# google/libultrahdr

Measured on AMD Instinct MI355X. Metric: Mpixels/s encode+decode (API-1 P010+YUV420, 4K), device-resident round trip, higher is better.
Workload: dtype f32; 1 GPU; API-1 3840x2160 round trip per step: encode (P010 HLG + YCbCr420 -> two-pass 3-ch gain map at scale 1, FDCT q95, Huffman: two JPEG scans) + decode (Huffman, IDCT, applyGainMap -> RGBA_F16 linear); frames resident in HBM

## Files before the change

libultrahdr_amd/csrc/api_entropy.cpp:

```cpp
#include "api_internal.h"

#include <condition_variable>
#include <functional>
#include <mutex>

uhdr_error_info_t uhdr_api::check_scan(const uhdr_hip_jpeg_scan_t* sc, bool need_coef, int* mcus_per_row, int* mcu_rows, int* blocks_per_mcu) {
  if (!sc) return err_status(UHDR_CODEC_INVALID_PARAM, "received nullptr for the scan description");
  if (sc->num_components != 1 && sc->num_components != 3)
    return err_status(UHDR_CODEC_INVALID_PARAM, "a scan has 1 or 3 components, received %d", sc->num_components);
  if (sc->w == 0 || sc->h == 0 || sc->w > 65535 || sc->h > 65535)
    return err_status(UHDR_CODEC_INVALID_PARAM, "image dimensions %ux%u are outside JPEG's 1..65535", sc->w, sc->h);
  int hmax = 1, vmax = 1, bpm = 0;
  for (int i = 0; i < sc->num_components; i++) {
    const int hs = sc->num_components == 1 ? 1 : sc->h_samp[i], vs = sc->num_components == 1 ? 1 : sc->v_samp[i];
    if (hs < 1 || hs > 2 || vs < 1 || vs > 2) return err_status(UHDR_CODEC_INVALID_PARAM, "component %d: sampling factors %dx%d not in {1, 2}", i, hs, vs);
    if (hs > hmax) hmax = hs;
    if (vs > vmax) vmax = vs;
    bpm += hs * vs;
    if (need_coef && (!sc->coef[i] || ((uintptr_t)sc->coef[i] & 15)))
      return err_status(UHDR_CODEC_INVALID_PARAM, "coefficient buffer %d is null or not 16-byte aligned", i);
    if (sc->blocks_w[i] < 1 || sc->blocks_h[i] < 1) return err_status(UHDR_CODEC_INVALID_PARAM, "component %d: empty block grid", i);
  }
  if (bpm > 10) return err_status(UHDR_CODEC_INVALID_PARAM, "an MCU holds at most 10 blocks (T.81 B.2.3), received %d", bpm);
  if (sc->num_components == 1) {
// ... 315 lines not shown
      if (n != 0 && !(n & 0x8000u) && (int)((n >> 8) & 31u) <= r) second = v_ac[next9];
    }
    out[2 * idx] = first;
    out[2 * idx + 1] = second;
  }
}

uhdr_error_info_t uhdr_hip_huffman_decode_dev(uhdr_hip_ctx_t* c, const uhdr_hip_jpeg_scan_t* sc, const uhdr_hip_huff_tables_t* tables,
                                              const uint8_t* data, size_t data_bytes) {
  if (!c) return err_status(UHDR_CODEC_INVALID_PARAM, "received nullptr for uhdr_hip context");
  if (!data || data_bytes == 0 || data_bytes > 0xFFFFFFF0ull) return err_status(UHDR_CODEC_INVALID_PARAM, "received no (or more than 4 GiB of) entropy-coded data");
  int mpr = 0, mrows = 0, bpm = 0;
  UHDR_TRY(check_scan(sc, true, &mpr, &mrows, &bpm));
  if (sc->restart_interval < 0 || sc->restart_interval > 65535) return err_status(UHDR_CODEC_INVALID_PARAM, "restart_interval %d out of range", sc->restart_interval);
  HIP_TRY(hipSetDevice(c->device));
  if (!c->d_huff) {
    std::vector<uint32_t> blob(host::jpeg_huff_code_tables());
    blob.resize((size_t)host::kHuffTabWords + 16);
    memcpy(blob.data() + host::kHuffTabWords, host::jpeg_zigzag_to_natural(), 64);
    HIP_TRY(hipMalloc((void**)&c->d_huff, blob.size() * sizeof(uint32_t)));
    HIP_TRY(hipMemcpyAsync(c->d_huff, blob.data(), blob.size() * sizeof(uint32_t), hipMemcpyHostToDevice, c->stream));
    HIP_TRY(hipStreamSynchronize(c->stream));
  }
  const DbgClock dbg;
  constexpr size_t kTabDec = 0, kTabFast = (sizeof(HuffDecTable) * 4 + 255) & ~(size_t)255,
                   kTabVal = (kTabFast + sizeof(HuffFastTable) * 8 + 255) & ~(size_t)255, kTabPair = kTabVal + (size_t)4 * kHuffValWords * 4,
                   kTabPairVal = kTabPair + (size_t)kHuffPairBlobWords * 4, kTabBytes = kTabPairVal + (size_t)kHuffPairValBlobWords * 4;
  {
    uint8_t key[4 * (17 + 256)];
    for (int t = 0; t < 4; t++) {
// ... 155 lines not shown
    const size_t o_sl = use_hyp ? take((size_t)nsub * (size_t)bpm * 8) : 0;
    const int max_pieces = [&] {
      const char* e = getenv("UHDR_HIP_HUFF_PIECES");
      const int v = e ? atoi(e) : 4;
      return (use_hyp && form2 && !rst_sync && v >= 1 && v <= 4) ? v : 1;
    }();
    const size_t o_ms = max_pieces > 1 ? take((size_t)nsub * kHuffHypSlots * (size_t)(max_pieces - 1) * 8) : 0;
    const size_t o_mc = max_pieces > 1 ? take((size_t)nsub * kHuffHypSlots * (size_t)(max_pieces - 1) * 2) : 0;
    const size_t o_pe = max_pieces > 1 ? take((size_t)nsub * (size_t)max_pieces * 8 + 64) : 0;
    const size_t o_pc = max_pieces > 1 ? take(((size_t)nsub * (size_t)max_pieces + 4) * 4) : 0;
    const size_t o_st2 = max_pieces > 1 ? take(((size_t)nsub * (size_t)max_pieces / 2048 + 4) * 4) : 0;
    const bool form3 = jblock_ok && attempts[0].levels > 0;
    const bool scratch2 = form2 && !form3;
    const size_t scan_bytes = scratch2 ? (size_t)total_blocks * 64 * sizeof(int16_t) : 0;
    const size_t o_cs = scratch2 ? take(scan_bytes + 256) : 0;
    UHDR_TRY(ensure(c->scratch[6], off));
    uint8_t* sb = (uint8_t*)c->scratch[6].p;
    HuffSyncArgs y;
    memset(&y, 0, sizeof y);
    y.clean = sb + o_clean;
    y.nbytes = (uint32_t)data_bytes;
    y.flags = (uint32_t*)(sb + o_flags);
    y.nstuffed = y.flags + 8;
    y.sub_bits = sub_bits;
    y.state[0] = (uint64_t*)(sb + o_s0); y.state[1] = (uint64_t*)(sb + o_s1);
    y.changed[0] = sb + o_c0; y.changed[1] = sb + o_c1;
    y.nblk = (uint32_t*)(sb + o_nblk);
    y.scan_tmp = (uint32_t*)(sb + o_st);
    y.dcd = (int*)(sb + o_dcd);
    y.total_blocks = total_blocks;
// ... 13 lines not shown
      y.first_blk[i] = j;
      for (int k = 0; k < a.hs[i] * a.vs[i] && j < 16; k++) y.comp_of[j++] = (uint8_t)i;
    }
    y.ftabs = (const HuffFastTable*)(tabs_dev + kTabFast);
    y.ttabs = y.ftabs + 4;
    y.vtabs = (const uint32_t*)(tabs_dev + kTabVal);
    y.ptabs = (const uint32_t*)(tabs_dev + kTabPair);
    y.pvtabs = (const uint32_t*)(tabs_dev + kTabPairVal);
    y.zigzag = a.zigzag;
    (void)o_ft; (void)o_vt;
    if (use_hyp) {
      y.strag_list = (uint32_t*)(sb + o_sl);
      y.strag_cap = nsub * (uint32_t)bpm;
    }
    if (scratch2) y.coef_scan = (int16_t*)(sb + o_cs);
    y.total_mcus = (uint32_t)a.total_mcus;
    const int main_levels_env = [&] { const char* e = getenv("UHDR_HIP_HUFF_MAIN_LEVELS"); return e ? atoi(e) : (sparse ? 1 : 2); }();
    if (j == bpm && bpm <= 16) {
      const bool fills_in_unstuff = attempts[0].levels > 0 && zero_bytes_sync % 16 == 0 && ff_bytes % 16 == 0 && zero_bytes_sync / 16 < 0xFFFFFFFFull &&
                                    ff_bytes / 16 < 0xFFFFFFFFull && !getenv("UHDR_HIP_HUFF_FILL_LAUNCHES");
      HuffInitFill init_fill;
      memset(&init_fill, 0, sizeof init_fill);
      if (fills_in_unstuff) {
        init_fill.zero_ptr = (uint4*)y.flags;
        init_fill.zero_vec = (uint32_t)(zero_bytes_sync / 16);
        init_fill.ff_ptr = (uint4*)y.state[0];
        init_fill.ff_vec = (uint32_t)(ff_bytes / 16);
      } else {
        HIP_TRY(hipMemsetAsync(y.flags, 0, zero_bytes_sync, c->stream));
      }
// ... 99 lines not shown
            fprintf(stderr, "uhdr_hip: rounds decode of %zu bytes, %u subsequences of %u bits (write form %d): %s\n", data_bytes, nsub_t, t.sub_bits,
                    y.coef_scan && !rst_sync ? 2 : 1, fl[4 + max_rounds % 3] == 0 ? "settled" : "NOT settled");
        }
      }
      const bool settled = hyp_done || fl[4 + max_rounds % 3] == 0;
      if (rst_sync && getenv("UHDR_HIP_HUFF_DEBUG"))
        fprintf(stderr, "uhdr_hip: restart file through the parallel decoder: %s, status bits %#x, %u markers dropped (%d expected), sequence sums %s\n",
                settled ? "settled" : "NOT settled", fl[1], fl[9], a.nseg - 1, fl[0] == fl[16] && fl[7] == fl[17] ? "equal" : "DIFFERENT");
      if (settled && rst_sync && ((fl[1] & 14u) != 0 || fl[9] != (uint32_t)(a.nseg - 1) || fl[0] != fl[16] || fl[7] != fl[17])) {
        for (int i = 0; i < a.ncomp; i++) HIP_TRY(hipMemsetAsync(a.coef[i], 0, zero_bytes[i], c->stream));
        coef_zeroed = true;
      } else if (settled) {
        if (fl[1] & 8u) return err_status(UHDR_CODEC_INVALID_PARAM, "corrupt entropy-coded data (the scan ends before its last block)");
        if (fl[1] & 2u) return err_status(UHDR_CODEC_INVALID_PARAM, "corrupt entropy-coded data (undefined Huffman code or a run past the end of a block)");
        sync_done = true;
      } else {
        if (a.nseg == 1 && !c->huff_serial_ok && data_bytes > (256u << 10)) {
          c->stats.entropy_decode_declined++;
          return err_status(UHDR_CODEC_UNSUPPORTED_FEATURE, "the parallel entropy decode did not settle in %d rounds; %zu bytes on one lane would take longer than the CPU", max_rounds, data_bytes);
        }
        for (int i = 0; i < a.ncomp; i++) HIP_TRY(hipMemsetAsync(a.coef[i], 0, zero_bytes[i], c->stream));
        coef_zeroed = true;
      }
    }
  }
  if (sync_done) {
    c->stats.entropy_decode_parallel++;
    return ok_status();
  }
  if (a.nseg == 1 && !c->huff_serial_ok && data_bytes > (256u << 10)) {
// ... 194 lines not shown
```

libultrahdr_amd/csrc/api_internal.h:

```cpp
#ifndef UHDR_HIP_API_INTERNAL_H
#define UHDR_HIP_API_INTERNAL_H

#pragma GCC visibility push(default)
#include "uhdr_hip.h"
#pragma GCC visibility pop

#include <cfloat>
#include <chrono>
#include <cmath>
#include <cstdarg>
#include <cstdio>
#include <cstring>
#include <atomic>
#include <functional>
#include <map>
#include <memory>
#include <string>
#include <thread>
#include <vector>
#include "exact_math.h"
#include "host_tables.h"
#include "uhdr_types.h"
#include "rccl_bind.h"

// ... 63 lines not shown
  float* d_pq_buckets = nullptr;
  float* d_hlg_buckets_pre = nullptr;
  float* d_pq_buckets_pre = nullptr;
  float* d_hlg_inv_ootf = nullptr;
  double* d_math = nullptr;
  float* h_tab[kTableSlots] = {};
  float* d_tab[kTableSlots] = {};
  size_t tab_cap[kTableSlots] = {};
  hipEvent_t tab_ev[kTableSlots] = {};
  std::string tab_key[kTableSlots];
  size_t tab_gamma_off[kTableSlots] = {};
  int tab_next = 0;
  DeviceBuf scratch[8];
  uhdr_hip_stats_t stats = {};
  bool huff_serial_ok = true;
  DeviceBuf huff_slots;
  bool huff_two_pass = false;
  bool huff_route_log = false;
  size_t huff_slots_refused = 0;
  DeviceBuf enc[3];
  uhdr_hip_ctx* aux = nullptr;
  struct AuxWorker* aux_worker = nullptr;
  DeviceBuf jpg[6];
  struct Resident {
    DeviceBuf buf;
    bool valid = false;
    uhdr_img_fmt_t fmt = UHDR_IMG_FMT_UNSPECIFIED;
    unsigned int w = 0, h = 0;
    const void* host[3] = {};
    unsigned int host_stride[3] = {};
// ... 146 lines not shown
```

libultrahdr_amd/csrc/api_jpeg.cpp:

```cpp
#include "api_internal.h"

void uhdr_hip_jpeg_quant_table(int quality, int is_chroma, uint16_t qt[64]) { host::jpeg_quant_table(quality, is_chroma, qt); }

int uhdr_hip_oetf_code_thresholds(uhdr_color_transfer_t ct, float thresholds[1024]) {
  if ((ct != UHDR_CT_HLG && ct != UHDR_CT_PQ) || !thresholds) return -1;
  const std::vector<float>& t = host::oetf_code_thresholds(ct);
  for (int i = 0; i < 1024; i++) thresholds[i] = t[(size_t)i];
  return 0;
}

uhdr_error_info_t uhdr_hip_selftest(uhdr_hip_ctx_t* c, int which, unsigned int arg0, unsigned int arg1, unsigned int seed, const float mm[6],
                                    unsigned long long out[8]) {
  if (!c) return err_status(UHDR_CODEC_INVALID_PARAM, "received nullptr for uhdr_hip context");
  if (!out || which < 0 || which > 7 || (which == 5 && !mm) || (which == 6 && (!mm || arg0 > 1)) ||
      ((which == 4 || which == 7) && (!mm || arg0 > 2 || arg1 < 1 || arg1 > 3 || arg0 >= arg1)) || (which == 2 && (arg0 < 1 || arg1 > 254 || arg0 > arg1)))
    return err_status(UHDR_CODEC_INVALID_PARAM, "bad self-test arguments");
  HIP_TRY(hipSetDevice(c->device));
  UHDR_TRY(upload_math(c));
  UHDR_TRY(ensure(c->affine, kAffineDevBytes));
  UHDR_TRY(ensure(c->exchange, 256));
  unsigned long long* d_out = (unsigned long long*)c->exchange.p;
  HIP_TRY(hipMemsetAsync(d_out, 0, 64, c->stream));
  if (which == 4) {
    MinmaxTableParams t;
// ... 979 lines not shown

uhdr_error_info_t uhdr_hip_jpeg_ycc_to_rgb(uhdr_hip_ctx_t* c, const uhdr_raw_image_t* ycc, int variant, uhdr_raw_image_t* rgb) {
  if (!c) return err_status(UHDR_CODEC_INVALID_PARAM, "received nullptr for uhdr_hip context");
  UHDR_TRY(check_jpeg_color(rgb, ycc, false));
  HIP_TRY(hipSetDevice(c->device));
  uhdr_raw_image_t tmp = *rgb;
  tmp.w = ycc->w; tmp.h = ycc->h;
  uhdr_raw_image_t ds, dd;
  UHDR_TRY(stage_in(c, 0, ycc, &ds, true));
  UHDR_TRY(stage_in(c, 1, &tmp, &dd, false));
  UHDR_TRY(uhdr_hip_jpeg_ycc_to_rgb_dev(c, &ds, variant, &dd));
  rgb->cg = dd.cg; rgb->ct = dd.ct; rgb->range = dd.range; rgb->w = dd.w; rgb->h = dd.h;
  return stage_out(c, &dd, rgb);
}

uhdr_error_info_t uhdr_hip_idct_dequant_rgb_dev(uhdr_hip_ctx_t* c, const int16_t* coef_y, const int16_t* coef_cb, const int16_t* coef_cr,
                                                int bw, int bh, const uint16_t qt_luma[64], const uint16_t qt_chroma[64], int variant,
                                                uhdr_raw_image_t* rgb) {
  if (!c) return err_status(UHDR_CODEC_INVALID_PARAM, "received nullptr for uhdr_hip context");
  if (!coef_y || !coef_cb || !coef_cr || !qt_luma || !qt_chroma || !rgb || !rgb->planes[0] || bw <= 0 || bh <= 0)
    return err_status(UHDR_CODEC_INVALID_PARAM, "received bad argument for idct_dequant_rgb");
  if (rgb->fmt != UHDR_IMG_FMT_24bppRGB888 && rgb->fmt != UHDR_IMG_FMT_32bppRGBA8888)
    return err_status(UHDR_CODEC_UNSUPPORTED_FEATURE, "idct_dequant_rgb expects UHDR_IMG_FMT_24bppRGB888 or UHDR_IMG_FMT_32bppRGBA8888. Received %d", rgb->fmt);
  if (variant != 0 && variant != 1) return err_status(UHDR_CODEC_INVALID_PARAM, "unknown libjpeg variant %d", variant);
  if (rgb->w == 0 || rgb->h == 0) return err_status(UHDR_CODEC_INVALID_PARAM, "image dimensions cannot be zero, received %ux%u", rgb->w, rgb->h);
  if ((rgb->w + 7) / 8 != (unsigned)bw || (rgb->h + 7) / 8 != (unsigned)bh)
    return err_status(UHDR_CODEC_INVALID_PARAM, "image %ux%u does not match a %dx%d block grid", rgb->w, rgb->h, bw, bh);
  if (rgb->stride[0] < rgb->w) return err_status(UHDR_CODEC_INVALID_PARAM, "stride (%u) cannot be less than width (%u)", rgb->stride[0], rgb->w);
  if (((uintptr_t)coef_y | (uintptr_t)coef_cb | (uintptr_t)coef_cr) & 15)
    return err_status(UHDR_CODEC_INVALID_PARAM, "coefficient buffers must be 16-byte aligned");
  for (int i = 0; i < 64; i++)
    if (qt_luma[i] == 0 || qt_chroma[i] == 0) return err_status(UHDR_CODEC_INVALID_PARAM, "quantization table entry %d is zero", i);
  HIP_TRY(hipSetDevice(c->device));
  rgb->range = UHDR_CR_FULL_RANGE;
  ProfScope ps(c, "idct_dequant");
  HIP_TRY(launch_idct_dequant_rgb(coef_y, coef_cb, coef_cr, bw, bh, qt_luma, qt_chroma, variant, view_mut_of(rgb), c->stream));
  return ok_status();
}

static uhdr_error_info_t jpeg_encode_impl(uhdr_hip_ctx_t* c, const uhdr_hip_jpeg_scan_t* scan, const uint16_t qtable[3][64],
                                          const uint8_t* const planes[3], const unsigned int strides[3], int rgb_channels, uint8_t* out,
                                          size_t out_capacity, size_t* out_bytes, bool image_edges) {
  if (!c) return err_status(UHDR_CODEC_INVALID_PARAM, "received nullptr for uhdr_hip context");
  if (!scan || !qtable || !planes || !strides || !out || !out_bytes) return err_status(UHDR_CODEC_INVALID_PARAM, "received nullptr argument for jpeg_encode_scan");
  if (rgb_channels != 0 && rgb_channels != 3 && rgb_channels != 4) return err_status(UHDR_CODEC_INVALID_PARAM, "rgb_channels is 0 (planes), 3 (RGB888) or 4 (RGBA8888), received %d", rgb_channels);
  uhdr_hip_jpeg_scan_t sc = *scan;
  const int nc = sc.num_components;
  int mpr = 0, mrows = 0, bpm = 0;
  UHDR_TRY(check_scan(&sc, false, &mpr, &mrows, &bpm));
  if (sc.restart_interval < 0 || sc.restart_interval * bpm > 64)
    return err_status(UHDR_CODEC_UNSUPPORTED_FEATURE, "restart_interval must be 0 (no markers) or in 1..%d for %d blocks per MCU, received %d", 64 / bpm, bpm, sc.restart_interval);
  HIP_TRY(hipSetDevice(c->device));
// ... 446 lines not shown
                                                                : "decode_api1_scans takes a 4:2:0 base image (the form JpegR writes); decode the scans with uhdr_hip_jpeg_decode_scan");
  UHDR_TRY(check_scan(&sm, false, &mpr, &mrows, &bpm));
  const int nm = sm.num_components;
  if (nm == 3 && (bpm != 3 || memcmp(map->qtable[1], map->qtable[2], sizeof map->qtable[1])))
    return err_status(UHDR_CODEC_UNSUPPORTED_FEATURE, "a three-channel gain map is a 4:4:4 scan with one chroma quantization table here");
  if (base_bytes == 0 || map_bytes == 0 || base_bytes > 0xFFFFFFF0ull || map_bytes > 0xFFFFFFF0ull) return err_status(UHDR_CODEC_INVALID_PARAM, "received no (or too much) entropy-coded data");
  HIP_TRY(hipSetDevice(c->device));
  for (int i = 0; i < 3; i++) {
    UHDR_TRY(ensure(c->jpg[1 + i], (size_t)sb.blocks_w[i] * sb.blocks_h[i] * 128));
    sb.coef[i] = (const int16_t*)c->jpg[1 + i].p;
  }
  size_t off = 0, o_map[3] = {0, 0, 0};
  for (int i = 0; i < nm; i++) { o_map[i] = off; off += ((size_t)sm.blocks_w[i] * sm.blocks_h[i] * 128 + 255) & ~(size_t)255; }
  UHDR_TRY(ensure(c->enc[0], off));
  for (int i = 0; i < nm; i++) sm.coef[i] = (const int16_t*)((const uint8_t*)c->enc[0].p + o_map[i]);
  c->huff_serial_ok = false;
  const uhdr_error_info_t hs = uhdr_hip_huffman_decode2_dev(c, &sb, tables_of(base), base_data, base_bytes, &sm, tables_of(map), map_data, map_bytes);
  c->huff_serial_ok = true;
  if (hs.error_code != UHDR_CODEC_OK) return hs;
  uhdr_raw_image_t gm;
  memset(&gm, 0, sizeof gm);
  gm.cg = map_cg;
  gm.ct = UHDR_CT_UNSPECIFIED;
  gm.range = UHDR_CR_FULL_RANGE;
  gm.w = sm.w;
  gm.h = sm.h;
  const size_t pitch_px = ((size_t)sm.w + 63) & ~(size_t)63;
  if (nm == 3) {
    gm.fmt = UHDR_IMG_FMT_32bppRGBA8888;
    UHDR_TRY(ensure(c->jpg[4], pitch_px * 4 * sm.h));
    gm.planes[0] = c->jpg[4].p;
    gm.stride[0] = (unsigned int)pitch_px;
    UHDR_TRY(uhdr_hip_idct_dequant_rgb_dev(c, sm.coef[0], sm.coef[1], sm.coef[2], sm.blocks_w[0], sm.blocks_h[0], map->qtable[0], map->qtable[1], libjpeg_variant, &gm));
  } else {
    gm.fmt = UHDR_IMG_FMT_8bppYCbCr400;
    const size_t pitch = ((size_t)sm.blocks_w[0] * 8 + 63) & ~(size_t)63;
    UHDR_TRY(ensure(c->jpg[4], pitch * (size_t)sm.blocks_h[0] * 8));
    gm.planes[0] = c->jpg[4].p;
    gm.stride[0] = (unsigned int)pitch;
    UHDR_TRY(uhdr_hip_idct_dequant_dev(c, sm.coef[0], sm.blocks_w[0], sm.blocks_h[0], map->qtable[0], (uint8_t*)c->jpg[4].p, pitch));
  }
  uhdr_hip_jpeg_coefficients_t bc;
  memset(&bc, 0, sizeof bc);
  for (int i = 0; i < 3; i++) {
    bc.coef[i] = sb.coef[i];
    bc.blocks_w[i] = sb.blocks_w[i];
    bc.blocks_h[i] = sb.blocks_h[i];
    memcpy(bc.qtable[i], base->qtable[i], sizeof bc.qtable[i]);
// ... 296 lines not shown
```

libultrahdr_amd/csrc/huffman_decode_sync.hip:

```cpp
#include <cstdio>
#include <cstdlib>
#include <cstring>

#include "lds_copy.h"
#include "wg_scan.h"
#include "uhdr_types.h"

namespace uhdr {
namespace {

constexpr int kChunk = 4096;
constexpr int kSyncBlock = 64;

__device__ __forceinline__ uint32_t rst_weight1(uint32_t at) { return (at * 2654435761u + 0x9e3779b9u) | 1u; }
__device__ __forceinline__ uint32_t rst_weight2(uint32_t at) { return ((at ^ (at >> 15)) * 0x85ebca6bu + 0xc2b2ae35u) | 1u; }
__device__ __forceinline__ bool is_stuffed(const uint8_t* __restrict__ d, uint32_t i) { return i > 0 && d[i] == 0 && d[i - 1] == 0xffu; }
__device__ __forceinline__ bool is_rst_first(const uint8_t* __restrict__ d, uint32_t i, uint32_t n) {
  return d[i] == 0xffu && i + 1 < n && (d[i + 1] & 0xf8u) == 0xd0u;
}
template <bool RST>
__device__ __forceinline__ bool is_dropped(const uint8_t* __restrict__ d, uint32_t i, uint32_t n) {
  if (is_stuffed(d, i)) return true;
  if (!RST) return false;
  return is_rst_first(d, i, n) || (i > 0 && (d[i] & 0xf8u) == 0xd0u && d[i - 1] == 0xffu);
// ... 650 lines not shown
  const uint16_t* S = &L.l2[0];
  const uint32_t limit = JB ? a.total_mcus : a.total_blocks;
  ptrdiff_t dA = 64, dB = 64, dC = 64;
  if (JB) {
    if (b >= bpm) b = 0;
    blk /= bpm;
    if (bpm == 3u) {
      const ptrdiff_t d0 = a.coef[1] - a.coef[0], d1 = a.coef[2] - a.coef[1], dl = a.coef[0] - a.coef[2] + 64;
      dA = b == 0 ? d0 : (b == 1 ? d1 : dl);
      dB = b == 0 ? d1 : (b == 1 ? dl : d0);
      dC = b == 0 ? dl : (b == 1 ? d0 : d1);
    }
  }
  uint32_t cls = JB ? (b ? 2u : 0u) : (((cpack >> (2u * b)) & 3u) ? 2u : 0u);
  int16_t* dst = JB ? a.coef[b] + (size_t)min(blk, limit) * 64 : a.coef_scan + (size_t)blk * 64;
  int16_t* pdst = dst;
  uint32_t pn1 = 0, pn2 = 0;
  int pv1 = 0, pv2 = 0;
  bool ps1 = false, ps2 = false;
  int left = (int)(end_bit - p);
  while (left > 0 && blk < limit) {
    r.fill();
    const uint32_t w16 = r.peek(16);
    const uint32_t ti = cls + (k ? 1u : 0u);
    const uint2 e = P[ti * (uint32_t)kHuffPairWords + (w16 >> (16 - kHuffPairBits))];
    uint32_t e1 = e.x, e2 = e.y;
    if (JB) {
      if (ps1) pdst[pn1] = (int16_t)pv1;
      if (ps2) pdst[pn2] = (int16_t)pv2;
    }
    if (__builtin_amdgcn_ballot_w64((e1 >> 31) != 0) != 0) {
      uint32_t s2 = S[((e1 >> 31) ? (e1 & 63u) : 0u) * 128u + (w16 & 127u)];
      s2 = s2 ? s2 : (16u | ((k ? 64u : 1u) << 5) | (1u << 16));
      e1 = (e1 >> 31) ? s2 : e1;
    }
    const uint32_t adv1 = e1 & 31u, kinc1 = (e1 >> 5) & 127u, sz1 = (e1 >> 12) & 15u;
    const bool two = e2 != 0u && k + kinc1 < 64u && left > (int)adv1;
    e2 = two ? e2 : 0u;
    const uint32_t adv2 = e2 & 31u, kinc2 = (e2 >> 5) & 127u, sz2 = (e2 >> 12) & 15u;
    const uint32_t adv = adv1 + adv2;
    const uint32_t bits = r.peek((int)adv);
    const uint32_t ext1 = (1u << sz1) - 1u, ext2 = (1u << sz2) - 1u;
    const uint32_t raw1 = (bits >> adv2) & ext1, raw2 = bits & ext2;
    const int v1 = (int)raw1 - (((raw1 << 1) > ext1) ? 0 : (int)ext1);
    const int v2 = (int)raw2 - (((raw2 << 1) > ext2) ? 0 : (int)ext2);
    const uint32_t zz1 = k + kinc1 - 1u, zz2 = zz1 + kinc2;
    const bool over1 = sz1 != 0 && zz1 > 63u, over2 = sz2 != 0 && zz2 > 63u;
    bad = bad || ((e1 >> 16) & 1u) != 0 || over1 || over2;
    if (JB) {
      pn1 = nat[zz1 & 63u];
      pn2 = nat[zz2 & 63u];
      pdst = dst;
      pv1 = v1; pv2 = v2;
      ps1 = sz1 != 0 && !over1;
      ps2 = sz2 != 0 && !over2;
    } else {
      if (sz1 != 0 && !over1) dst[zz1] = (int16_t)v1;
      if (sz2 != 0 && !over2) dst[zz2] = (int16_t)v2;
    }
    r.skip((int)adv);
    left -= (int)adv;
    k += kinc1 + kinc2;
    if (k >= 64u) {
      k = 0;
      if constexpr (JB) {
        const bool last = b + 1u == bpm;
        dst += dA;
        const ptrdiff_t t = dA;
        dA = dB; dB = dC; dC = t;
        b = last ? 0u : b + 1u;
        nblk++;
        blk += last ? 1u : 0u;
        cls = b ? 2u : 0u;
      } else {
        b++;
        nblk++;
        blk++;
        dst += 64;
        if (b == bpm) b = 0;
        cls = ((cpack >> (2u * b)) & 3u) ? 2u : 0u;
      }
    }
  }
  if (JB) {
    if (ps1) pdst[pn1] = (int16_t)pv1;
    if (ps2) pdst[pn2] = (int16_t)pv2;
  }
  if (bad) atomicOr(a.flags + 1, 2u);
}
template <bool JB>
__global__ __launch_bounds__(256) void sync_write2_kernel(const HuffSyncArgs a, int final_buf) {
  extern __shared__ __attribute__((aligned(16))) uint32_t s_dyn[];
  Write2Lds& L = *(Write2Lds*)s_dyn;
  uint32_t* s_stage_all = s_dyn + sizeof(Write2Lds) / 4;
  static_assert(sizeof(Write2Lds) == kHuffPairValBlobWords * 4, "Write2Lds is one copy of the host's blob");
  copy_words_to_lds(s_dyn, a.pvtabs, (uint32_t)kHuffPairValBlobWords, threadIdx.x, blockDim.x);
  const uint32_t i = blockIdx.x * blockDim.x + threadIdx.x;
  const uint32_t nclean = a.nbytes - *a.nstuffed, nbits = nclean * 8u;
  const uint32_t nsub = (nbits + a.sub_bits - 1) / a.sub_bits;
  const uint32_t cshift = 31u - (uint32_t)__builtin_clz(a.sub_bits >> 3);
// ... 717 lines not shown
    uint32_t* dst = (uint32_t*)(base + (size_t)(ent & 0x3fffffffu) * 64);
    dst[lane & 31u] = lo | (hi << 16);
  }
}
__device__ __forceinline__ int16_t* dc_term3(const HuffSyncArgs& a, uint32_t t, int& c) {
  const uint32_t n = (uint32_t)a.ncomp, m = t / n;
  c = (int)(t - m * n);
  int16_t* base = c == 0 ? a.coef[0] : (c == 1 ? a.coef[1] : a.coef[2]);
  return base + (size_t)m * 64;
}
__global__ __launch_bounds__(kPlaceChunk) void dc_partial3_kernel(const HuffSyncArgs a, int* __restrict__ partial) {
  __shared__ int s_sum[3 * (kPlaceChunk / 64)];
  const int tid = (int)threadIdx.x;
  const uint32_t t = blockIdx.x * (uint32_t)kPlaceChunk + (uint32_t)tid;
  int v[3] = {0, 0, 0};
  if (t < a.total_blocks) {
    int c;
    const int16_t* d = dc_term3(a, t, c);
    v[c] = *d;
  }
  dc_chunk_scan(v, s_sum, tid);
  if (tid == kPlaceChunk - 1) { partial[blockIdx.x * 3] = v[0]; partial[blockIdx.x * 3 + 1] = v[1]; partial[blockIdx.x * 3 + 2] = v[2]; }
}
__global__ __launch_bounds__(kPlaceChunk) void dc_apply3_kernel(const HuffSyncArgs a, const int* __restrict__ partial, int self_prefix) {
  __shared__ int s_sum[3 * (kPlaceChunk / 64)];
  const int tid = (int)threadIdx.x;
  const uint32_t t = blockIdx.x * (uint32_t)kPlaceChunk + (uint32_t)tid;
  int v[3] = {0, 0, 0};
  int c = 0;
  int16_t* d = nullptr;
  if (t < a.total_blocks) {
    d = dc_term3(a, t, c);
    v[c] = *d;
  }
  int carry[3];
  if (self_prefix) {
    int part[3] = {0, 0, 0};
    for (uint32_t i = (uint32_t)tid; i < blockIdx.x; i += (uint32_t)kPlaceChunk) {
      part[0] += partial[i * 3];
      part[1] += partial[i * 3 + 1];
      part[2] += partial[i * 3 + 2];
    }
    wg_incl_scan<kPlaceChunk, 3>(part, s_sum, carry);
  } else {
    carry[0] = partial[blockIdx.x * 3];
    carry[1] = partial[blockIdx.x * 3 + 1];
    carry[2] = partial[blockIdx.x * 3 + 2];
  }
  dc_chunk_scan(v, s_sum, tid);
  if (d) *d = (int16_t)((c == 0 ? carry[0] : (c == 1 ? carry[1] : carry[2])) + v[c]);
}
__global__ __launch_bounds__(1024) void dc_scan_partials_kernel(int* __restrict__ partial, int nchunks) {
  __shared__ int s_sum[3 * 16];
  const int tid = (int)threadIdx.x;
  const int per = (nchunks + 1023) / 1024, lo = min(tid * per, nchunks), hi = min(lo + per, nchunks);
  int v[3] = {0, 0, 0};
  for (int i = lo; i < hi; i++)
    for (int c = 0; c < 3; c++) v[c] += partial[i * 3 + c];
  int own[3] = {v[0], v[1], v[2]};
  dc_block_scan(v, s_sum, tid);
  int run[3] = {v[0] - own[0], v[1] - own[1], v[2] - own[2]};
  for (int i = lo; i < hi; i++)
    for (int c = 0; c < 3; c++) {
      const int x = partial[i * 3 + c];
      partial[i * 3 + c] = run[c];
// ... 292 lines not shown
```

libultrahdr_amd/csrc/idct_core.h:

```cpp
#pragma once
#include "jdct_fix.h"
#include "uhdr_types.h"

namespace uhdr {
namespace idct {

template <bool M24>
__device__ __forceinline__ int mulc(int a, int c) {
  if constexpr (M24) return __mul24(a, c);
  else return (int)((uint32_t)a * (uint32_t)c);
}
template <int PASS, bool M24>
__device__ __forceinline__ void idct_1d(const int in[8], int out[8]) {
  constexpr int sh = PASS == 0 ? 13 - 2 : 13 + 2 + 3;
  constexpr uint32_t fudge = (1u << (sh - 1)) + (PASS == 1 ? (512u << 18) : 0u);
  int z2 = in[2], z3 = in[6];
  int z1 = mulc<M24>(z2 + z3, FIX_0_541196100);
  int tmp2 = z1 + mulc<M24>(z3, -FIX_1_847759065);
  int tmp3 = z1 + mulc<M24>(z2, FIX_0_765366865);
  z2 = in[0]; z3 = in[4];
  int tmp0 = (int)(((uint32_t)(z2 + z3) << 13) + fudge);
  int tmp1 = (int)(((uint32_t)(z2 - z3) << 13) + fudge);
  const int tmp10 = tmp0 + tmp3, tmp13 = tmp0 - tmp3, tmp11 = tmp1 + tmp2, tmp12 = tmp1 - tmp2;
  tmp0 = in[7]; tmp1 = in[5]; tmp2 = in[3]; tmp3 = in[1];
// ... 11 lines not shown
  z3 += z5; z4 += z5;
  tmp0 += z1 + z3; tmp1 += z2 + z4; tmp2 += z2 + z3; tmp3 += z1 + z4;
  const int sum[8] = {tmp10 + tmp3, tmp11 + tmp2, tmp12 + tmp1, tmp13 + tmp0, tmp13 - tmp0, tmp12 - tmp1, tmp11 - tmp2, tmp10 - tmp3};
#pragma unroll
  for (int k = 0; k < 8; k++) {
    if constexpr (PASS == 0) {
      out[k] = sum[k] >> sh;
    } else {
      const int t = (int)(((uint32_t)sum[k] >> 18) & 1023u) - 384;
      out[k] = min(max(t, 0), 255);
    }
  }
}

__device__ __forceinline__ void load_dequant_row(const int16_t* __restrict__ coef, int bw, int by, int bx, int rr,
                                                 const int q[8], int v[8], int& big, bool row_ok = true) {
  if (bx < bw && row_ok) {
    const uint4 raw = *(const uint4*)(coef + ((size_t)by * bw + bx) * 64 + rr * 8);
    const uint32_t w4[4] = {raw.x, raw.y, raw.z, raw.w};
#pragma unroll
    for (int c = 0; c < 4; c++) {
      v[2 * c] = __mul24((int)(int16_t)(w4[c] & 0xffff), q[2 * c]);
      v[2 * c + 1] = __mul24((int)(int16_t)(w4[c] >> 16), q[2 * c + 1]);
    }
    const int mx = max(max(max(v[0], v[1]), max(v[2], v[3])), max(max(v[4], v[5]), max(v[6], v[7])));
    const int mn = min(min(min(v[0], v[1]), min(v[2], v[3])), min(min(v[4], v[5]), min(v[6], v[7])));
    big |= (int)(mx > 8191) | (int)(mn < -8191);
  } else {
#pragma unroll
    for (int c = 0; c < 8; c++) v[c] = 0;
  }
}

__device__ __forceinline__ void idct_wave(int* ws, const int v[8], int big, int rr, int rb, uint32_t s[8]) {
// ... 26 lines not shown
```

libultrahdr_amd/csrc/jpeg_decode.hip:

```cpp
#include "coef_tile.h"
#include "uhdr_types.h"
#include "upsample_core.h"

namespace uhdr {
namespace {

using namespace idct;
using namespace upsample;

constexpr int kBlock = 256;

struct DequantArgs {
  uint16_t q[64];
};

__global__ __launch_bounds__(kBlock) void idct_dequant_kernel(const int16_t* __restrict__ coef, int bw, int bh,
                                                              const DequantArgs qa, uint8_t* __restrict__ plane,
                                                              size_t stride) {
  __shared__ int s_ws[kBlock / 64][8 * 8 * 9];
  const int lane = threadIdx.x & 63, wv = threadIdx.x >> 6;
  int* ws = s_ws[wv];
  const int groups_x = (bw + 7) >> 3, total = groups_x * bh;
  const int gwave = blockIdx.x * (kBlock / 64) + wv, nwaves = gridDim.x * (kBlock / 64);
  const int rr = lane >> 3, rb = lane & 7;
// ... 110 lines not shown
                                 p.p[2][(size_t)y * p.stride[2] + j], p.k_cr_g, p.k_cb_g);
      dst[j * BPP] = (uint8_t)px; dst[j * BPP + 1] = (uint8_t)(px >> 8); dst[j * BPP + 2] = (uint8_t)(px >> 16);
      if constexpr (BPP == 4) dst[j * BPP + 3] = 255;
    }
  }
}

struct IdctRgbArgs {
  const int16_t* coef[3];
  uint8_t* rgb;
  size_t pitch;
  uint32_t w, h;
  int bw, bh;
  int k_cr_g, k_cb_g;
  uint16_t q[2][64];
};

template <int BPP>
__global__ __launch_bounds__(kBlock) void idct_dequant_rgb_kernel(const IdctRgbArgs a) {
  __shared__ int s_ws[kBlock / 64][8 * 8 * 9];
  const int lane = threadIdx.x & 63, wv = threadIdx.x >> 6;
  int* ws = s_ws[wv];
  const int bw = a.bw;
  const int groups_x = (bw + 7) >> 3, total = groups_x * a.bh;
  const int gwave = blockIdx.x * (kBlock / 64) + wv, nwaves = gridDim.x * (kBlock / 64);
  const int rr = lane >> 3, rb = lane & 7;
  int ql[8], qc[8];
#pragma unroll
  for (int c = 0; c < 8; c++) { ql[c] = a.q[0][rr * 8 + c]; qc[c] = a.q[1][rr * 8 + c]; }
  const bool vec_ok = ((a.pitch | (uintptr_t)a.rgb) & (BPP == 4 ? 15 : 7)) == 0;

  for (int t = gwave; t < total; t += nwaves) {
    const int by = t / groups_x, gx = t - by * groups_x;
    const int bx = gx * 8 + rb;
    int vy[8], vb[8], vr[8];
    int big_y = 0, big_b = 0, big_r = 0;
    load_dequant_row(a.coef[0], bw, by, bx, rr, ql, vy, big_y);
    load_dequant_row(a.coef[1], bw, by, bx, rr, qc, vb, big_b);
    load_dequant_row(a.coef[2], bw, by, bx, rr, qc, vr, big_r);
    uint32_t sy[8], sb[8], sr[8];
    idct_wave(ws, vy, big_y, rr, rb, sy);
    idct_wave(ws, vb, big_b, rr, rb, sb);
    idct_wave(ws, vr, big_r, rr, rb, sr);
    const uint32_t y = (uint32_t)(by * 8 + rr), x0 = (uint32_t)bx * 8;
    if (bx < bw && y < a.h && x0 < a.w) {
      uint32_t px[8];
#pragma unroll
      for (int c = 0; c < 8; c++) px[c] = ycc_px(sy[c], sb[c], sr[c], a.k_cr_g, a.k_cb_g);
      store_px8<BPP>(a.rgb + (size_t)y * a.pitch + (size_t)x0 * BPP, px, x0, a.w, vec_ok);
    }
  }
}

inline bool al(const void* p, size_t a) { return ((uintptr_t)p % a) == 0; }

}

hipError_t launch_idct_dequant(const int16_t* coef, int bw, int bh, const uint16_t* qt_host, uint8_t* plane,
                               size_t stride, hipStream_t s) {
  DequantArgs qa;
  for (int i = 0; i < 64; i++) qa.q[i] = qt_host[i];
  const int total = ((bw + 7) / 8) * bh;
  const int grid = resident_grid((uint32_t)(total + 3) / 4, 8);
  hipLaunchKernelGGL(idct_dequant_kernel, dim3(grid), dim3(kBlock), 0, s, coef, bw, bh, qa, plane, stride);
  return hipGetLastError();
}

hipError_t launch_idct_dequant_rgb(const int16_t* coef_y, const int16_t* coef_cb, const int16_t* coef_cr, int bw, int bh,
                                   const uint16_t* qt_luma_host, const uint16_t* qt_chroma_host, int variant,
                                   const ImageViewMut& rgb, hipStream_t s) {
  IdctRgbArgs a = {};
  a.coef[0] = coef_y; a.coef[1] = coef_cb; a.coef[2] = coef_cr;
  a.rgb = (uint8_t*)rgb.p[0];
  const int bpp = rgb.fmt == UHDR_IMG_FMT_32bppRGBA8888 ? 4 : 3;
  a.pitch = (size_t)rgb.stride[0] * bpp;
  a.w = rgb.w; a.h = rgb.h; a.bw = bw; a.bh = bh;
  ycc_green_constants(variant, &a.k_cr_g, &a.k_cb_g);
  for (int i = 0; i < 64; i++) { a.q[0][i] = qt_luma_host[i]; a.q[1][i] = qt_chroma_host[i]; }
  const int total = ((bw + 7) / 8) * bh;
  const int grid = resident_grid((uint32_t)(total + 3) / 4, 8);
  if (bpp == 4) hipLaunchKernelGGL((idct_dequant_rgb_kernel<4>), dim3(grid), dim3(kBlock), 0, s, a);
  else hipLaunchKernelGGL((idct_dequant_rgb_kernel<3>), dim3(grid), dim3(kBlock), 0, s, a);
  return hipGetLastError();
}

hipError_t launch_jpeg_rgb_to_ycc(const ImageView& rgb, const ImageViewMut& ycc, hipStream_t s) {
  JpegColorParams p = {};
  p.rgb = (const uint8_t*)rgb.p[0];
  p.w = rgb.w; p.h = rgb.h; p.rgb_stride_px = rgb.stride[0];
  p.bpp = rgb.fmt == UHDR_IMG_FMT_32bppRGBA8888 ? 4 : 3;
  for (int c = 0; c < 3; c++) { p.po[c] = (uint8_t*)ycc.p[c]; p.stride[c] = ycc.stride[c]; }
  const bool vec = (p.w % 4 == 0) && al(p.rgb, p.bpp == 4 ? 16 : 4) && ((size_t)p.rgb_stride_px * p.bpp) % (p.bpp == 4 ? 16 : 4) == 0 &&
                   al(p.po[0], 4) && al(p.po[1], 4) && al(p.po[2], 4) && p.stride[0] % 4 == 0 && p.stride[1] % 4 == 0 && p.stride[2] % 4 == 0;
  const uint32_t per_row = vec ? p.w / 4 : p.w;
  const int grid = resident_grid(((per_row + kBlock - 1) / kBlock) * p.h, 8);
  if (p.bpp == 4) {
    if (vec) hipLaunchKernelGGL((jpeg_rgb_to_ycc_kernel<4, true>), dim3(grid), dim3(kBlock), 0, s, p);
// ... 31 lines not shown
```

libultrahdr_amd/csrc/uhdr_types.h:

```cpp
#pragma once
#include <hip/hip_runtime.h>
#include <stdint.h>

#include "device_math.h"
#include "uhdr_hip.h"

namespace uhdr {

struct ImageView {
  const void* p[3];
  uint32_t stride[3];
  uint32_t w, h;
  int fmt;
  int range;
};
struct ImageViewMut {
  void* p[3];
  uint32_t stride[3];
  uint32_t w, h;
  int fmt;
  int range;
};

constexpr int kSrgbN = 1024;
// ... 326 lines not shown
  const uint32_t* ptabs;
  const uint32_t* pvtabs;
  const uint8_t* zigzag;
  int hyp_h, hyp_levels;
  uint64_t* hyp_state;
  uint8_t* hyp_map;
  uint16_t* hyp_cnt;
  int hyp_hist;
  int hyp_main_levels;
  int strag_levels;
  uint32_t* strag_list;
  uint32_t strag_cap;
  int16_t* coef_scan;
  int write_form;
  uint32_t total_mcus;
  uint4* zero_ptr[3];
  uint32_t zero_vec[3];
  int pieces;
  uint64_t* mid_state;
  uint16_t* mid_cnt;
  uint64_t* pend;
  uint32_t* pcnt;
  const uint32_t* rst_map;
  uint32_t rst_blocks;
  int* dc_seg;
  uint32_t* rst_partial;
  uint32_t rst_chunks;
};
constexpr int kHuffHypSlots = 48;
constexpr int kHuffFlagStragglers = 20;
// ... 9 lines not shown
  uint32_t ff_vec;
};
hipError_t launch_huffman_unstuff(const uint8_t* data, uint32_t nbytes, uint32_t* chunk_counts, uint32_t* nstuffed_dev, uint8_t* clean, hipStream_t s,
                                  uint32_t* rst_map, uint32_t* rst_partial, const HuffInitFill* fill = nullptr);
hipError_t launch_huffman_decode_sync(const HuffSyncArgs& a, int max_rounds, int* dc_partial, int* final_buf, hipStream_t s);
void launch_profile_mark(hipStream_t s);
int huff_marker_chunks(uint64_t nbytes);
int huff_place_chunk();
hipError_t launch_stray_marker_check(const uint8_t* data, uint32_t nbytes, uint32_t* flag, hipStream_t s);
hipError_t launch_huffman_decode(const HuffDecArgs& a, uint32_t* counts, uint32_t* starts, uint32_t* ends, hipStream_t s);

hipError_t launch_idct_dequant(const int16_t* coef, int bw, int bh, const uint16_t* qt_host, uint8_t* plane,
                               size_t stride, hipStream_t s);
hipError_t launch_idct_dequant_rgb(const int16_t* coef_y, const int16_t* coef_cb, const int16_t* coef_cr, int bw, int bh,
                                   const uint16_t* qt_luma_host, const uint16_t* qt_chroma_host, int variant,
                                   const ImageViewMut& rgb, hipStream_t s);
size_t upsample_scratch_bytes(const int bw[3], const int bh[3]);
hipError_t launch_idct_upsample_rgb(const int16_t* const coef[3], const int bw[3], const int bh[3], const uint16_t* const qt_host[3],
                                    int variant, int vsamp, const ImageViewMut& rgb, uint8_t* chroma_scratch, hipStream_t s);
hipError_t launch_jpeg_rgb_to_ycc(const ImageView& rgb, const ImageViewMut& ycc, hipStream_t s);
hipError_t launch_jpeg_ycc_to_rgb(const ImageView& ycc, const ImageViewMut& rgb, int variant, hipStream_t s);

}
```

Before: 12910 Mpixels/s.

## Keep Huffman DC terms in a dense side array and patch them in IDCT

```diff
diff --git a/libultrahdr_amd/csrc/api_entropy.cpp b/libultrahdr_amd/csrc/api_entropy.cpp
--- a/libultrahdr_amd/csrc/api_entropy.cpp
+++ b/libultrahdr_amd/csrc/api_entropy.cpp
@@ -353,6 +353,7 @@
   UHDR_TRY(check_scan(sc, true, &mpr, &mrows, &bpm));
   if (sc->restart_interval < 0 || sc->restart_interval > 65535) return err_status(UHDR_CODEC_INVALID_PARAM, "restart_interval %d out of range", sc->restart_interval);
   HIP_TRY(hipSetDevice(c->device));
+  c->huff_dc_dense = nullptr;
   if (!c->d_huff) {
     std::vector<uint32_t> blob(host::jpeg_huff_code_tables());
     blob.resize((size_t)host::kHuffTabWords + 16);
@@ -538,6 +539,7 @@
     const bool scratch2 = form2 && !form3;
     const size_t scan_bytes = scratch2 ? (size_t)total_blocks * 64 * sizeof(int16_t) : 0;
     const size_t o_cs = scratch2 ? take(scan_bytes + 256) : 0;
+    const size_t o_dd = form3 ? take((size_t)total_blocks * sizeof(int16_t)) : 0;
     UHDR_TRY(ensure(c->scratch[6], off));
     uint8_t* sb = (uint8_t*)c->scratch[6].p;
     HuffSyncArgs y;
@@ -581,6 +583,10 @@
       y.strag_cap = nsub * (uint32_t)bpm;
     }
     if (scratch2) y.coef_scan = (int16_t*)(sb + o_cs);
+    if (form3) {
+      y.dc_dense = (int16_t*)(sb + o_dd);
+      y.dc_no_scatter = c->huff_dc_side ? 1 : 0;
+    }
     y.total_mcus = (uint32_t)a.total_mcus;
     const int main_levels_env = [&] { const char* e = getenv("UHDR_HIP_HUFF_MAIN_LEVELS"); return e ? atoi(e) : (sparse ? 1 : 2); }();
     if (j == bpm && bpm <= 16) {
@@ -710,6 +716,7 @@
         if (fl[1] & 8u) return err_status(UHDR_CODEC_INVALID_PARAM, "corrupt entropy-coded data (the scan ends before its last block)");
         if (fl[1] & 2u) return err_status(UHDR_CODEC_INVALID_PARAM, "corrupt entropy-coded data (undefined Huffman code or a run past the end of a block)");
         sync_done = true;
+        if (hyp_done && y.write_form == 3 && y.dc_no_scatter) c->huff_dc_dense = y.dc_dense;
       } else {
         if (a.nseg == 1 && !c->huff_serial_ok && data_bytes > (256u << 10)) {
           c->stats.entropy_decode_declined++;
diff --git a/libultrahdr_amd/csrc/api_internal.h b/libultrahdr_amd/csrc/api_internal.h
--- a/libultrahdr_amd/csrc/api_internal.h
+++ b/libultrahdr_amd/csrc/api_internal.h
@@ -101,6 +101,8 @@
   DeviceBuf scratch[8];
   uhdr_hip_stats_t stats = {};
   bool huff_serial_ok = true;
+  bool huff_dc_side = false;
+  const int16_t* huff_dc_dense = nullptr;
   DeviceBuf huff_slots;
   bool huff_two_pass = false;
   bool huff_route_log = false;
diff --git a/libultrahdr_amd/csrc/api_jpeg.cpp b/libultrahdr_amd/csrc/api_jpeg.cpp
--- a/libultrahdr_amd/csrc/api_jpeg.cpp
+++ b/libultrahdr_amd/csrc/api_jpeg.cpp
@@ -1017,9 +1017,9 @@
   return stage_out(c, &dd, rgb);
 }
 
-uhdr_error_info_t uhdr_hip_idct_dequant_rgb_dev(uhdr_hip_ctx_t* c, const int16_t* coef_y, const int16_t* coef_cb, const int16_t* coef_cr,
-                                                int bw, int bh, const uint16_t qt_luma[64], const uint16_t qt_chroma[64], int variant,
-                                                uhdr_raw_image_t* rgb) {
+static uhdr_error_info_t idct_dequant_rgb_impl(uhdr_hip_ctx_t* c, const int16_t* coef_y, const int16_t* coef_cb, const int16_t* coef_cr, int bw, int bh,
+                                               const uint16_t qt_luma[64], const uint16_t qt_chroma[64], int variant, uhdr_raw_image_t* rgb,
+                                               const int16_t* dc_dense) {
   if (!c) return err_status(UHDR_CODEC_INVALID_PARAM, "received nullptr for uhdr_hip context");
   if (!coef_y || !coef_cb || !coef_cr || !qt_luma || !qt_chroma || !rgb || !rgb->planes[0] || bw <= 0 || bh <= 0)
     return err_status(UHDR_CODEC_INVALID_PARAM, "received bad argument for idct_dequant_rgb");
@@ -1037,8 +1037,13 @@
   HIP_TRY(hipSetDevice(c->device));
   rgb->range = UHDR_CR_FULL_RANGE;
   ProfScope ps(c, "idct_dequant");
-  HIP_TRY(launch_idct_dequant_rgb(coef_y, coef_cb, coef_cr, bw, bh, qt_luma, qt_chroma, variant, view_mut_of(rgb), c->stream));
-  return ok_status();
+  HIP_TRY(launch_idct_dequant_rgb(coef_y, coef_cb, coef_cr, bw, bh, qt_luma, qt_chroma, variant, view_mut_of(rgb), c->stream, dc_dense));
+  return ok_status();
+}
+uhdr_error_info_t uhdr_hip_idct_dequant_rgb_dev(uhdr_hip_ctx_t* c, const int16_t* coef_y, const int16_t* coef_cb, const int16_t* coef_cr,
+                                                int bw, int bh, const uint16_t qt_luma[64], const uint16_t qt_chroma[64], int variant,
+                                                uhdr_raw_image_t* rgb) {
+  return idct_dequant_rgb_impl(c, coef_y, coef_cb, coef_cr, bw, bh, qt_luma, qt_chroma, variant, rgb, nullptr);
 }
 
 static uhdr_error_info_t jpeg_encode_impl(uhdr_hip_ctx_t* c, const uhdr_hip_jpeg_scan_t* scan, const uint16_t qtable[3][64],
@@ -1515,10 +1520,15 @@
   for (int i = 0; i < nm; i++) { o_map[i] = off; off += ((size_t)sm.blocks_w[i] * sm.blocks_h[i] * 128 + 255) & ~(size_t)255; }
   UHDR_TRY(ensure(c->enc[0], off));
   for (int i = 0; i < nm; i++) sm.coef[i] = (const int16_t*)((const uint8_t*)c->enc[0].p + o_map[i]);
+  uhdr_hip_ctx* x = nullptr;
+  UHDR_TRY(aux_context(c, &x));
+  x->huff_dc_side = nm == 3;
   c->huff_serial_ok = false;
   const uhdr_error_info_t hs = uhdr_hip_huffman_decode2_dev(c, &sb, tables_of(base), base_data, base_bytes, &sm, tables_of(map), map_data, map_bytes);
   c->huff_serial_ok = true;
+  x->huff_dc_side = false;
   if (hs.error_code != UHDR_CODEC_OK) return hs;
+  const int16_t* map_dc = nm == 3 ? x->huff_dc_dense : nullptr;
   uhdr_raw_image_t gm;
   memset(&gm, 0, sizeof gm);
   gm.cg = map_cg;
@@ -1532,7 +1542,7 @@
     UHDR_TRY(ensure(c->jpg[4], pitch_px * 4 * sm.h));
     gm.planes[0] = c->jpg[4].p;
     gm.stride[0] = (unsigned int)pitch_px;
-    UHDR_TRY(uhdr_hip_idct_dequant_rgb_dev(c, sm.coef[0], sm.coef[1], sm.coef[2], sm.blocks_w[0], sm.blocks_h[0], map->qtable[0], map->qtable[1], libjpeg_variant, &gm));
+    UHDR_TRY(idct_dequant_rgb_impl(c, sm.coef[0], sm.coef[1], sm.coef[2], sm.blocks_w[0], sm.blocks_h[0], map->qtable[0], map->qtable[1], libjpeg_variant, &gm, map_dc));
   } else {
     gm.fmt = UHDR_IMG_FMT_8bppYCbCr400;
     const size_t pitch = ((size_t)sm.blocks_w[0] * 8 + 63) & ~(size_t)63;
diff --git a/libultrahdr_amd/csrc/huffman_decode_sync.hip b/libultrahdr_amd/csrc/huffman_decode_sync.hip
--- a/libultrahdr_amd/csrc/huffman_decode_sync.hip
+++ b/libultrahdr_amd/csrc/huffman_decode_sync.hip
@@ -688,7 +688,9 @@
   }
   uint32_t cls = JB ? (b ? 2u : 0u) : (((cpack >> (2u * b)) & 3u) ? 2u : 0u);
   int16_t* dst = JB ? a.coef[b] + (size_t)min(blk, limit) * 64 : a.coef_scan + (size_t)blk * 64;
+  int16_t* dcp = JB ? a.dc_dense + ((size_t)min(blk, limit) * bpm + b) : nullptr;
   int16_t* pdst = dst;
+  int16_t* pdst1 = dst;
   uint32_t pn1 = 0, pn2 = 0;
   int pv1 = 0, pv2 = 0;
   bool ps1 = false, ps2 = false;
@@ -699,8 +701,9 @@
     const uint32_t ti = cls + (k ? 1u : 0u);
     const uint2 e = P[ti * (uint32_t)kHuffPairWords + (w16 >> (16 - kHuffPairBits))];
     uint32_t e1 = e.x, e2 = e.y;
+    const bool dc1 = JB && k == 0u;
     if (JB) {
-      if (ps1) pdst[pn1] = (int16_t)pv1;
+      if (ps1) pdst1[pn1] = (int16_t)pv1;
       if (ps2) pdst[pn2] = (int16_t)pv2;
     }
     if (__builtin_amdgcn_ballot_w64((e1 >> 31) != 0) != 0) {
@@ -725,8 +728,9 @@
       pn1 = nat[zz1 & 63u];
       pn2 = nat[zz2 & 63u];
       pdst = dst;
+      pdst1 = dc1 ? dcp : dst;
       pv1 = v1; pv2 = v2;
-      ps1 = sz1 != 0 && !over1;
+      ps1 = dc1 || (sz1 != 0 && !over1);
       ps2 = sz2 != 0 && !over2;
     } else {
       if (sz1 != 0 && !over1) dst[zz1] = (int16_t)v1;
@@ -740,6 +744,7 @@
       if constexpr (JB) {
         const bool last = b + 1u == bpm;
         dst += dA;
+        dcp++;
         const ptrdiff_t t = dA;
         dA = dB; dB = dC; dC = t;
         b = last ? 0u : b + 1u;
@@ -757,7 +762,7 @@
     }
   }
   if (JB) {
-    if (ps1) pdst[pn1] = (int16_t)pv1;
+    if (ps1) pdst1[pn1] = (int16_t)pv1;
     if (ps2) pdst[pn2] = (int16_t)pv2;
   }
   if (bad) atomicOr(a.flags + 1, 2u);
@@ -1505,11 +1510,7 @@
   const int tid = (int)threadIdx.x;
   const uint32_t t = blockIdx.x * (uint32_t)kPlaceChunk + (uint32_t)tid;
   int v[3] = {0, 0, 0};
-  if (t < a.total_blocks) {
-    int c;
-    const int16_t* d = dc_term3(a, t, c);
-    v[c] = *d;
-  }
+  if (t < a.total_blocks) v[t % (uint32_t)a.ncomp] = a.dc_dense[t];
   dc_chunk_scan(v, s_sum, tid);
   if (tid == kPlaceChunk - 1) { partial[blockIdx.x * 3] = v[0]; partial[blockIdx.x * 3 + 1] = v[1]; partial[blockIdx.x * 3 + 2] = v[2]; }
 }
@@ -1519,10 +1520,9 @@
   const uint32_t t = blockIdx.x * (uint32_t)kPlaceChunk + (uint32_t)tid;
   int v[3] = {0, 0, 0};
   int c = 0;
-  int16_t* d = nullptr;
   if (t < a.total_blocks) {
-    d = dc_term3(a, t, c);
-    v[c] = *d;
+    c = (int)(t % (uint32_t)a.ncomp);
+    v[c] = a.dc_dense[t];
   }
   int carry[3];
   if (self_prefix) {
@@ -1539,7 +1539,13 @@
     carry[2] = partial[blockIdx.x * 3 + 2];
   }
   dc_chunk_scan(v, s_sum, tid);
-  if (d) *d = (int16_t)((c == 0 ? carry[0] : (c == 1 ? carry[1] : carry[2])) + v[c]);
+  if (t >= a.total_blocks) return;
+  const int16_t dc = (int16_t)((c == 0 ? carry[0] : (c == 1 ? carry[1] : carry[2])) + v[c]);
+  a.dc_dense[t] = dc;
+  if (!a.dc_no_scatter) {
+    int cc;
+    *dc_term3(a, t, cc) = dc;
+  }
 }
 __global__ __launch_bounds__(1024) void dc_scan_partials_kernel(int* __restrict__ partial, int nchunks) {
   __shared__ int s_sum[3 * 16];
diff --git a/libultrahdr_amd/csrc/idct_core.h b/libultrahdr_amd/csrc/idct_core.h
--- a/libultrahdr_amd/csrc/idct_core.h
+++ b/libultrahdr_amd/csrc/idct_core.h
@@ -49,10 +49,10 @@
 }
 
 __device__ __forceinline__ void load_dequant_row(const int16_t* __restrict__ coef, int bw, int by, int bx, int rr,
-                                                 const int q[8], int v[8], int& big, bool row_ok = true) {
+                                                 const int q[8], int v[8], int& big, bool row_ok = true, bool dc_put = false, uint32_t dc = 0) {
   if (bx < bw && row_ok) {
     const uint4 raw = *(const uint4*)(coef + ((size_t)by * bw + bx) * 64 + rr * 8);
-    const uint32_t w4[4] = {raw.x, raw.y, raw.z, raw.w};
+    const uint32_t w4[4] = {dc_put ? (raw.x & 0xffff0000u) | (dc & 0xffffu) : raw.x, raw.y, raw.z, raw.w};
 #pragma unroll
     for (int c = 0; c < 4; c++) {
       v[2 * c] = __mul24((int)(int16_t)(w4[c] & 0xffff), q[2 * c]);
diff --git a/libultrahdr_amd/csrc/jpeg_decode.hip b/libultrahdr_amd/csrc/jpeg_decode.hip
--- a/libultrahdr_amd/csrc/jpeg_decode.hip
+++ b/libultrahdr_amd/csrc/jpeg_decode.hip
@@ -148,9 +148,10 @@
   int bw, bh;
   int k_cr_g, k_cb_g;
   uint16_t q[2][64];
+  const int16_t* dc_dense;
 };
 
-template <int BPP>
+template <int BPP, bool DENSE>
 __global__ __launch_bounds__(kBlock) void idct_dequant_rgb_kernel(const IdctRgbArgs a) {
   __shared__ int s_ws[kBlock / 64][8 * 8 * 9];
   const int lane = threadIdx.x & 63, wv = threadIdx.x >> 6;
@@ -169,9 +170,20 @@
     const int bx = gx * 8 + rb;
     int vy[8], vb[8], vr[8];
     int big_y = 0, big_b = 0, big_r = 0;
-    load_dequant_row(a.coef[0], bw, by, bx, rr, ql, vy, big_y);
-    load_dequant_row(a.coef[1], bw, by, bx, rr, qc, vb, big_b);
-    load_dequant_row(a.coef[2], bw, by, bx, rr, qc, vr, big_r);
+    uint32_t dc_yb = 0, dc_r = 0;
+    const bool dc_put = DENSE && rr == 0;
+    if constexpr (DENSE) {
+      if (rr == 0 && bx < bw) {
+        uint32_t m = (uint32_t)(by * bw + bx);
+        asm volatile("" : "+v"(m));
+        const uint32_t m3 = m * 3u;
+        dc_yb = (uint32_t)(uint16_t)a.dc_dense[m3] | ((uint32_t)(uint16_t)a.dc_dense[m3 + 1u] << 16);
+        dc_r = (uint16_t)a.dc_dense[m3 + 2u];
+      }
+    }
+    load_dequant_row(a.coef[0], bw, by, bx, rr, ql, vy, big_y, true, dc_put, dc_yb);
+    load_dequant_row(a.coef[1], bw, by, bx, rr, qc, vb, big_b, true, dc_put, dc_yb >> 16);
+    load_dequant_row(a.coef[2], bw, by, bx, rr, qc, vr, big_r, true, dc_put, dc_r);
     uint32_t sy[8], sb[8], sr[8];
     idct_wave(ws, vy, big_y, rr, rb, sy);
     idct_wave(ws, vb, big_b, rr, rb, sb);
@@ -202,9 +214,10 @@
 
 hipError_t launch_idct_dequant_rgb(const int16_t* coef_y, const int16_t* coef_cb, const int16_t* coef_cr, int bw, int bh,
                                    const uint16_t* qt_luma_host, const uint16_t* qt_chroma_host, int variant,
-                                   const ImageViewMut& rgb, hipStream_t s) {
+                                   const ImageViewMut& rgb, hipStream_t s, const int16_t* dc_dense) {
   IdctRgbArgs a = {};
   a.coef[0] = coef_y; a.coef[1] = coef_cb; a.coef[2] = coef_cr;
+  a.dc_dense = dc_dense;
   a.rgb = (uint8_t*)rgb.p[0];
   const int bpp = rgb.fmt == UHDR_IMG_FMT_32bppRGBA8888 ? 4 : 3;
   a.pitch = (size_t)rgb.stride[0] * bpp;
@@ -213,8 +226,11 @@
   for (int i = 0; i < 64; i++) { a.q[0][i] = qt_luma_host[i]; a.q[1][i] = qt_chroma_host[i]; }
   const int total = ((bw + 7) / 8) * bh;
   const int grid = resident_grid((uint32_t)(total + 3) / 4, 8);
-  if (bpp == 4) hipLaunchKernelGGL((idct_dequant_rgb_kernel<4>), dim3(grid), dim3(kBlock), 0, s, a);
-  else hipLaunchKernelGGL((idct_dequant_rgb_kernel<3>), dim3(grid), dim3(kBlock), 0, s, a);
+  if (dc_dense) {
+    if (bpp != 4) return hipErrorInvalidValue;
+    hipLaunchKernelGGL((idct_dequant_rgb_kernel<4, true>), dim3(grid), dim3(kBlock), 0, s, a);
+  } else if (bpp == 4) hipLaunchKernelGGL((idct_dequant_rgb_kernel<4, false>), dim3(grid), dim3(kBlock), 0, s, a);
+  else hipLaunchKernelGGL((idct_dequant_rgb_kernel<3, false>), dim3(grid), dim3(kBlock), 0, s, a);
   return hipGetLastError();
 }
 
diff --git a/libultrahdr_amd/csrc/uhdr_types.h b/libultrahdr_amd/csrc/uhdr_types.h
--- a/libultrahdr_amd/csrc/uhdr_types.h
+++ b/libultrahdr_amd/csrc/uhdr_types.h
@@ -364,6 +364,8 @@
   int16_t* coef_scan;
   int write_form;
   uint32_t total_mcus;
+  int16_t* dc_dense;
+  int dc_no_scatter;
   uint4* zero_ptr[3];
   uint32_t zero_vec[3];
   int pieces;
@@ -403,7 +405,7 @@
                                size_t stride, hipStream_t s);
 hipError_t launch_idct_dequant_rgb(const int16_t* coef_y, const int16_t* coef_cb, const int16_t* coef_cr, int bw, int bh,
                                    const uint16_t* qt_luma_host, const uint16_t* qt_chroma_host, int variant,
-                                   const ImageViewMut& rgb, hipStream_t s);
+                                   const ImageViewMut& rgb, hipStream_t s, const int16_t* dc_dense = nullptr);
 size_t upsample_scratch_bytes(const int bw[3], const int bh[3]);
 hipError_t launch_idct_upsample_rgb(const int16_t* const coef[3], const int bw[3], const int bh[3], const uint16_t* const qt_host[3],
                                     int variant, int vsamp, const ImageViewMut& rgb, uint8_t* chroma_scratch, hipStream_t s);
```

New measurement: 13230 Mpixels/s, median of 6. +2.5%, better.
